# hinike/cairo

Hardware: AMD Instinct MI355X
Metric: encoded Mpixels/s (p-frame, q=16) at 1/2/4/8 MI355X; bit-exact vs ref (higher is better)
Workload: dtype int16

## Files before the change

### cairo_amd/__init__.py

```python
from __future__ import annotations

import ctypes
import os
from dataclasses import dataclass

import numpy as np

_HERE = os.path.dirname(os.path.abspath(__file__))
LIB_PATH = os.path.join(_HERE, "_lib", "libcairo_amd.so")

BLOCK_DESC = np.dtype(
    [
        ("block_type", "<u4"),
        ("prediction_target", "u1"),
        ("pad", "u1"),
        ("motion_x", "<i2"),
        ("motion_y", "<i2"),
        ("sp_pred", "u1"),
        ("sp_amount", "u1"),
        ("sp_index", "u1"),
        ("q_index", "u1"),
        ("variance", "<i2"),
    ]
)
# ... 292 lines not shown
        self.wmb, self.hmb = self.wa // 16, self.ha // 16
        p = ctypes.c_void_p()
        _ck(self.L.cairo_ctx_create_ex(width, height, ring, device, stages, ctypes.byref(p)), "cairo_ctx_create")
        self.h = p
        self._keep = {}

    def close(self) -> None:
        if self.h:
            self.L.cairo_ctx_destroy(self.h)
            self.h = None

    def __del__(self):
        try:
            self.close()
        except Exception:
            pass

    @property
    def stages(self) -> int:
        return int(self.L.cairo_ctx_stages(self.h))

    def submit(self, rgb, index: int, inter: bool, quality: int, on_device: bool = False,
               fmt: int = FMT_RGB24, pitch: int = 0) -> int:
        t = ctypes.c_int()
        ptr = rgb if on_device else _host_frame_fmt(rgb, fmt, self.width, self.height, pitch)
        if fmt == FMT_RGB24 and not pitch:
            _ck(
                self.L.cairo_ctx_submit(self.h, ptr, int(on_device), index, int(inter), quality, ctypes.byref(t)),
                "cairo_ctx_submit",
            )
        else:
            _ck(self.L.cairo_ctx_submit_fmt(self.h, ptr, int(on_device), fmt, pitch, index, int(inter), quality,
                                            ctypes.byref(t)), "cairo_ctx_submit_fmt")
        if not on_device:
            self._keep[t.value] = rgb
        return t.value

    def wait(self, ticket: int, copy: bool = True) -> FrameOutputs:
        r = _FrameResult()
        st = self.L.cairo_ctx_wait(self.h, ticket, ctypes.byref(r))
        if st != EVX_SUCCESS:
            raise CairoError("cairo_ctx_wait", st, self.timeout_info() if st == EVX_ERROR_HARDWAREFAIL else None)
        self._keep.pop(ticket, None)
        return self._outputs(r, copy)

    ACCT_FIELDS = ("coder_tasks", "coder_total", "coder_group_wait", "coder_window", "coder_search", "coder_inter",
                   "coder_dequeue", "coder_mbs", "helper_tasks", "helper_total", "helper_wait", "helper_deblock",
                   "helper_search", "helper_catchup", "helper_dequeue", "helper_chunks",
                   "win_bytes", "win_spec_unused_bytes", "zero_mv_bytes", "gran_poll_bytes", "rec_poll_bytes",
                   "win_stages", "searched_tasks", "inter_tasks", "coder_xform", "coder_publish", "coder_drain",
                   "coder_vm0", "coder_records", "coder_prebarrier", "coder_store_tail",
                   "search_eval", "search_barrier", "search_select", "subpel_eval", "subpel_barrier",
                   "subpel_select", "db_inputs", "db_filter", "db_write",
                   "search_passes", "search_mbs_2pass", "search_mbs_3pass", "search_mbs_4pass")

    def read_acct(self, reset: bool = False) -> dict:
        w = np.zeros(len(self.ACCT_FIELDS), np.uint64)
        _ck(self.L.cairo_ctx_read_acct(self.h, _ptr(w), len(w), int(reset)), "cairo_ctx_read_acct")
        return {k: int(w[i]) for i, k in enumerate(self.ACCT_FIELDS)}

    def timeout_info(self) -> dict | None:
        w = np.zeros(16, np.int32)
        _ck(self.L.cairo_ctx_timeout_info(self.h, _ptr(w), 16), "cairo_ctx_timeout_info")
        if not w[0]:
            return None
        d = {k: int(w[i]) for i, k in enumerate(TIMEOUT_FIELDS)}
        d["kind"] = WAIT_KINDS.get(d["kind"], str(d["kind"]))
        d["seen"] = (d.pop("seen_hi") & 0xFFFFFFFF) << 32 | (d.pop("seen_lo") & 0xFFFFFFFF)
        return d

    def _outputs(self, r, copy: bool) -> FrameOutputs:
        ny, nc = r.wa * r.ha, (r.wa // 2) * (r.ha // 2)
        mbs = r.wmb * r.hmb
        has_coef = bool(r.coef_y)
        feed = _view(r.feed, np.uint32, (r.feed_bits + 31) // 32) if r.feed_status == FEED_VALID else None
        out = FrameOutputs(
            _view(r.block_table, BLOCK_DESC, mbs),
            _view(r.coef_y, np.int16, ny).reshape(r.ha, r.wa) if has_coef else None,
            _view(r.coef_u, np.int16, nc).reshape(r.ha // 2, r.wa // 2) if has_coef else None,
            _view(r.coef_v, np.int16, nc).reshape(r.ha // 2, r.wa // 2) if has_coef else None,
            feed, int(r.feed_bits), int(r.feed_status),
        )
        if copy:
            cp = lambda a: None if a is None else a.copy()
            out = FrameOutputs(cp(out.table), cp(out.coef_y), cp(out.coef_u), cp(out.coef_v), cp(out.feed),
                               out.feed_bits, out.feed_status)
        return out

    def set_outputs(self, outputs: int) -> None:
        _ck(self.L.cairo_ctx_set_outputs(self.h, outputs), "cairo_ctx_set_outputs")

    def fetch_coef(self, ticket: int):
        r = _FrameResult()
        _ck(self.L.cairo_ctx_fetch_coef(self.h, ticket, ctypes.byref(r)), "cairo_ctx_fetch_coef")
        ny, nc = self.wa * self.ha, (self.wa // 2) * (self.ha // 2)
        return (_view(r.coef_y, np.int16, ny).reshape(self.ha, self.wa).copy(),
                _view(r.coef_u, np.int16, nc).reshape(self.ha // 2, self.wa // 2).copy(),
                _view(r.coef_v, np.int16, nc).reshape(self.ha // 2, self.wa // 2).copy())

    def set_metrics(self, sse: bool = True, ssim: bool = True, keep_recon: bool = False, flags: int | None = None) -> None:
        if flags is None:
            flags = (METRIC_SSE if sse else 0) | (METRIC_SSIM if ssim else 0) | (KEEP_RECON if keep_recon else 0)
        _ck(self.L.cairo_ctx_set_metrics(self.h, flags), "cairo_ctx_set_metrics")

    def frame_metrics(self, ticket: int) -> dict:
        m = _FrameMetrics()
        _ck(self.L.cairo_ctx_frame_metrics(self.h, ticket, ctypes.byref(m)), "cairo_ctx_frame_metrics")
# ... 498 lines not shown
```

### cairo_amd/csrc/kernels.h

```cpp
#pragma once

#include <hip/hip_runtime.h>
#include <stdint.h>

#include "evx_defs.h"

namespace cairo {

struct PlaneSet {
  int16_t* y;
  int16_t* u;
  int16_t* v;
};

__host__ __device__ inline PlaneSet ring_slot(int16_t* base, size_t slot_elems, int wa, int ha,
                                              int k) {
  PlaneSet p;
  p.y = base + (size_t)k * slot_elems;
  p.u = p.y + (size_t)wa * ha;
  p.v = p.u + (size_t)(wa / 2) * (ha / 2);
  return p;
}

constexpr int kGranulesPerMB = 192;
// ... 2 lines not shown
__host__ __device__ inline uint32_t pack_inter_desc(const BlockDesc& d) {
  return (d.block_type & 7u) | ((uint32_t)(d.prediction_target & 3) << 3) | ((uint32_t)(d.sp_pred & 1) << 5) |
         ((uint32_t)(d.sp_amount & 1) << 6) | ((uint32_t)(d.sp_index & 15) << 7) |
         (((uint32_t)d.motion_x & 0x7Fu) << 11) | (((uint32_t)d.motion_y & 0x7Fu) << 18);
}
__host__ __device__ inline BlockDesc unpack_inter_desc(uint32_t w) {
  BlockDesc d;
  d.block_type = w & 7u;
  d.prediction_target = (uint8_t)((w >> 3) & 3);
  d.pad = 0;
  d.sp_pred = (uint8_t)((w >> 5) & 1);
  d.sp_amount = (uint8_t)((w >> 6) & 1);
  d.sp_index = (uint8_t)((w >> 7) & 15);
  d.motion_x = (int16_t)((int32_t)(w << 14) >> 25);
  d.motion_y = (int16_t)((int32_t)(w << 7) >> 25);
  d.q_index = 0;
  d.variance = 0;
  return d;
}

constexpr int kStampPhases = 12;
constexpr int kDbStamps = 256;
constexpr int kIStamps = 12;
__host__ __device__ inline size_t stamp_frame_words(int wmb, int hmb) {
  return (size_t)wmb * hmb * kStampPhases + (size_t)hmb * kDbStamps;
}

struct TimeoutInfo {
  static constexpr int kKind = 0;
  static constexpr int kEpoch = 1;
  static constexpr int kIndex = 2;
  static constexpr int kRow = 3;
  static constexpr int kMember = 4;
  static constexpr int kNeed = 5;
  static constexpr int kOn = 6;
  static constexpr int kSeenLo = 7;
  static constexpr int kSeenHi = 8;
  static constexpr int kClaim = 9;
  static constexpr int kWords = 16;
};
enum TimeoutKind : int32_t {
  kWaitRecords = 1,
  kWaitGranule = 2,
  kWaitPrevProgress = 3,
  kWaitRowAbove = 4,
  kWaitBatch = 5,
  kWaitInjected = 6,
  kWaitHostMark = 9,
};

#ifndef CAIRO_ACCT
#define CAIRO_ACCT 0
#endif
constexpr int kAcctShards = 64, kAcctWords = 44;
struct Acct {
  static constexpr int kCoderTasks = 0, kCoderTotal = 1, kCoderGroupWait = 2, kCoderWindow = 3, kCoderSearch = 4,
                       kCoderInter = 5, kCoderDequeue = 6, kCoderMBs = 7;
  static constexpr int kHelperTasks = 8, kHelperTotal = 9, kHelperWait = 10, kHelperDeblock = 11, kHelperSearch = 12,
                       kHelperCatchup = 13, kHelperDequeue = 14, kHelperChunks = 15;
  static constexpr int kWinBytes = 16, kWinSpecUnused = 17, kZeroMvBytes = 18, kGranPollBytes = 19,
                       kRecPollBytes = 20, kWinStages = 21, kSearchedTasks = 22, kInterTasks = 23;
  static constexpr int kCoderXform = 24, kCoderPublish = 25, kCoderDrain = 26;
  static constexpr int kCoderVm0 = 27, kCoderRecords = 28, kCoderPreBarrier = 29;
  static constexpr int kCoderStoreTail = 30;
  static constexpr int kSrchEval = 31, kSrchBarrier = 32, kSrchSelect = 33, kSubEval = 34, kSubBarrier = 35,
                       kSubSelect = 36;
  static constexpr int kDbInputs = 37, kDbFilter = 38, kDbWrite = 39;
  static constexpr int kSrchPasses = 40, kSrchPasses2 = 41, kSrchPasses3 = 42, kSrchPasses4 = 43;
};

#ifndef CAIRO_MAX_BATCH
#define CAIRO_MAX_BATCH 48
#endif
constexpr int kMaxBatch = CAIRO_MAX_BATCH;
constexpr int kMaxGroup = 16;
constexpr int kMaxPush = kMaxRing;

struct FrameDesc {
  const uint8_t* rgb;
  const uint8_t* host_rgb;
  int index;
  int inter;
  int quality;
  uint32_t epoch;
  int slot;
  int decode;
  PlaneSet recon[kMaxRing];
  PlaneSet stale;
  PlaneSet coef;
  PlaneSet push[kMaxPush];
  int npush;
  PlaneSet coef_prev;
  uint64_t* progress;
  const uint64_t* prev_progress;
  const uint64_t* prev2_progress;
  int sys;
  int member;
  const BlockDesc* host_table;
  const int16_t* host_coef;
};

struct FrameArgs {
  int wa, ha;
  int w, h;
  int wmb, hmb;
  int ring;
  int index, inter, quality;
  int decode;
  uint32_t epoch;
  PlaneSet in;
  PlaneSet coef;
  PlaneSet coef_prev;
  PlaneSet recon[kMaxRing];
  PlaneSet stale;
  PlaneSet push[kMaxPush];
  int npush;
  BlockDesc* table;
  BlockDesc* inter_desc;
  void* reserved0;
  uint64_t* granules;
  int32_t* err;
// ... 105 lines not shown
```

### cairo_amd/csrc/kernels.hip

```cpp
#include "kernels.h"

namespace cairo {

typedef const __attribute__((address_space(4))) FrameArgs FA;
#define RECON_AT(a, k)                                                                   \
  ((k) == 1 ? planes((a).recon[1]) : (k) == 2 ? planes((a).recon[2]) : (k) == 3 ? planes((a).recon[3]) \
                                                                              : planes((a).recon[0]))
__host__ __device__ inline PlaneSet planes(const __attribute__((address_space(4))) PlaneSet& p) {
  PlaneSet r;
  r.y = p.y;
  r.u = p.u;
  r.v = p.v;
  return r;
}


__constant__ int16_t kLut8[64] = {
    128, 128,  128,  128,  128,  128,  128,  128,
    126, 106,  71,   25,   -25,  -71,  -106, -126,
    118, 49,   -49,  -118, -118, -49,  49,   118,
    106, -25,  -126, -71,  71,   126,  25,   -106,
    91,  -91,  -91,  91,   91,   -91,  -91,  91,
    71,  -126, 25,   106,  -106, -25,  126,  -71,
    49,  -118, 118,  -49,  -49,  118,  -118, 49,
// ... 39 lines not shown
    sMagDcC[q] = div_magic(chroma_dc_scale(q));
  } else if (t < 192) {
    sMagQmIntra[t - 128] = div_magic(kQmIntra[t - 128]);
    sMagQmInter[t - 128] = div_magic(kQmInter[t - 128]);
  }
  __syncthreads();
}


__device__ __forceinline__ int wave_sum(int v) {
  v += __builtin_amdgcn_mov_dpp(v, 0x128, 0xF, 0xF, false);
  v += __builtin_amdgcn_mov_dpp(v, 0x124, 0xF, 0xF, false);
  v += __builtin_amdgcn_mov_dpp(v, 0x122, 0xF, 0xF, false);
  v += __builtin_amdgcn_mov_dpp(v, 0x121, 0xF, 0xF, false);
  return __builtin_amdgcn_readlane(v, 0) + __builtin_amdgcn_readlane(v, 16) +
         __builtin_amdgcn_readlane(v, 32) + __builtin_amdgcn_readlane(v, 48);
}
__device__ __forceinline__ int wave_max(int v) {
  v = max(v, __builtin_amdgcn_mov_dpp(v, 0x128, 0xF, 0xF, false));
  v = max(v, __builtin_amdgcn_mov_dpp(v, 0x124, 0xF, 0xF, false));
  v = max(v, __builtin_amdgcn_mov_dpp(v, 0x122, 0xF, 0xF, false));
  v = max(v, __builtin_amdgcn_mov_dpp(v, 0x121, 0xF, 0xF, false));
  return max(max(__builtin_amdgcn_readlane(v, 0), __builtin_amdgcn_readlane(v, 16)),
             max(__builtin_amdgcn_readlane(v, 32), __builtin_amdgcn_readlane(v, 48)));
}

__device__ __forceinline__ int lane_id() { return threadIdx.x & 63; }

__device__ __forceinline__ void trace(int32_t* t, int k, int v) {
  if (t && threadIdx.x == 0)
    __hip_atomic_store(&t[blockIdx.x * 4 + k], v, __ATOMIC_RELAXED, __HIP_MEMORY_SCOPE_SYSTEM);
}

__device__ __forceinline__ int16_t* pick(const PlaneSet& p, int pl) {
  int16_t* const y = p.y;
  int16_t* const u = p.u;
  int16_t* const v = p.v;
  return pl == 0 ? y : (pl == 1 ? u : v);
}

__device__ __forceinline__ int fresh(int v) {
  asm volatile("" : "+v"(v));
  return v;
}

__device__ __forceinline__ int uni(int v) { return __builtin_amdgcn_readfirstlane(v); }

__device__ __forceinline__ void stamp(FA& a, int mb, int k) {
  if (a.stamps && threadIdx.x == 0)
    a.stamps[(size_t)mb * kStampPhases + k] = __builtin_amdgcn_s_memrealtime();
}

__device__ __forceinline__ uint64_t acct_now() { return CAIRO_ACCT ? __builtin_amdgcn_s_memrealtime() : 0; }
__device__ __forceinline__ void acct_add(uint64_t* acct, int k, uint64_t v) {
  if (CAIRO_ACCT && acct && threadIdx.x == 0)
    __hip_atomic_fetch_add(&acct[(blockIdx.x & (kAcctShards - 1)) * kAcctWords + k], v, __ATOMIC_RELAXED,
                           __HIP_MEMORY_SCOPE_AGENT);
}

__device__ __forceinline__ uint64_t tagged(uint32_t epoch, int cols) {
  return ((uint64_t)epoch << 32) | (uint32_t)cols;
}
__device__ __forceinline__ uint64_t progress_at(const uint64_t* p) {
  return __hip_atomic_load(p, __ATOMIC_RELAXED, __HIP_MEMORY_SCOPE_AGENT);
}
__device__ __forceinline__ uint64_t progress_peer(bool sys, const uint64_t* p) {
  return sys ? __hip_atomic_load(p, __ATOMIC_RELAXED, __HIP_MEMORY_SCOPE_SYSTEM)
             : __hip_atomic_load(p, __ATOMIC_RELAXED, __HIP_MEMORY_SCOPE_AGENT);
}
__device__ __forceinline__ void acquire_fence(bool sys) {
  if (sys)
    __builtin_amdgcn_fence(__ATOMIC_ACQUIRE, "");
  else
    __builtin_amdgcn_fence(__ATOMIC_ACQUIRE, "agent");
}

constexpr int kWaitSleep = 2, kGranSleep = 1;

__device__ __attribute__((noinline)) void report_timeout(int32_t* err, int32_t* sticky, int kind, uint32_t epoch,
                                                         int index, int row, int member, int need, int on,
                                                         uint64_t seen) {
  __hip_atomic_store(err, 1, __ATOMIC_RELAXED, __HIP_MEMORY_SCOPE_AGENT);
  int32_t none = 0;
  if (!__hip_atomic_compare_exchange_strong(sticky + TimeoutInfo::kClaim, &none, 1, __ATOMIC_RELAXED,
                                            __ATOMIC_RELAXED, __HIP_MEMORY_SCOPE_AGENT))
    return;
  const int32_t w[8] = {(int32_t)epoch, index, row, member, need, on, (int32_t)(uint32_t)seen, (int32_t)(seen >> 32)};
  for (int k = 0; k < 8; k++) __hip_atomic_store(sticky + 1 + k, w[k], __ATOMIC_RELAXED, __HIP_MEMORY_SCOPE_AGENT);
  __hip_atomic_store(sticky + TimeoutInfo::kKind, kind, __ATOMIC_RELEASE, __HIP_MEMORY_SCOPE_SYSTEM);
}
__device__ __forceinline__ void report_timeout(FA& a, int kind, int row, int need, int on, uint64_t seen) {
  report_timeout(a.err, a.sticky, kind, a.epoch, a.index, row, a.member, need, on, seen);
}

__device__ __forceinline__ void wait_records(FA& a, int row, int group) {
  int32_t* word = &a.inter_done[row * a.ng + group];
  int v = __hip_atomic_load(word, __ATOMIC_RELAXED, __HIP_MEMORY_SCOPE_AGENT);
  if (v >= a.nref) return;
  uint64_t t0 = __builtin_amdgcn_s_memrealtime();
  while ((v = __hip_atomic_load(word, __ATOMIC_RELAXED, __HIP_MEMORY_SCOPE_AGENT)) < a.nref) {
    if (__hip_atomic_load(a.err, __ATOMIC_RELAXED, __HIP_MEMORY_SCOPE_AGENT)) return;
    __builtin_amdgcn_s_sleep(kWaitSleep);
    if (__builtin_amdgcn_s_memrealtime() - t0 > 200000000ull) {
      report_timeout(a, kWaitRecords, row, a.nref, group, (uint32_t)v);
      return;
    }
// ... 587 lines not shown
  if (lane >= 48) return;
  const PlaneSet in = planes(a.in);
  const int px = x * kMB, py = r * kMB;
  const int16_t* gsrc = lane < 32 ? in.y + (size_t)(py + (lane >> 1)) * a.wa + px + 8 * (lane & 1)
                                  : pick(in, 1 + ((lane - 32) >> 3)) +
                                        (size_t)((py >> 1) + (lane & 7)) * (a.wa >> 1) + (px >> 1);
  __builtin_amdgcn_global_load_lds((const void*)gsrc, (lds_void*)dst, 16, 0, 0);
}

__device__ __forceinline__ Px6 src_px_lds(const InterLds& L, int wave) {
  const int l = threadIdx.x & 63;
  const int16_t* m = L.src[wave];
  Px6 p;
  const int16_t* y = &m[(l >> 2) * 16 + (l & 3) * 4];
  p.y0 = y[0], p.y1 = y[1], p.y2 = y[2], p.y3 = y[3];
  p.u = m[256 + (l >> 3) * 8 + (l & 7)];
  p.v = m[320 + (l >> 3) * 8 + (l & 7)];
  return p;
}
__device__ __forceinline__ SrcRow src_rows_lds(const InterLds& L, int wave, int i) {
  const uint32_t* m = (const uint32_t*)L.src[wave];
  SrcRow s;
#pragma unroll
  for (int k = 0; k < 8; k++) s.y[k] = m[i * 8 + k] ^ 0x80008000u;
  const int co = (i >> 1) * 4 + (i & 1) * 2;
  s.u[0] = m[128 + co] ^ 0x80008000u, s.u[1] = m[128 + co + 1] ^ 0x80008000u;
  s.v[0] = m[160 + co] ^ 0x80008000u, s.v[1] = m[160 + co + 1] ^ 0x80008000u;
  return s;
}

__device__ __forceinline__ void zero_mv_older(FA& a, int r, int g, InterLds& L) {
  const int wave = threadIdx.x >> 6, x = 4 * g + wave;
  acct_add(a.acct, Acct::kZeroMvBytes, 768ull * (a.nref - 1) * (uint64_t)min(4, a.wmb - 4 * g));
  if (x >= a.wmb) return;
  const int px = x * kMB, py = r * kMB;
  const Px6 src = src_px_lds(L, wave);
  Px6 ref[kMaxRing - 1];
#pragma unroll
  for (int off = 2; off < kMaxRing; off++)
    if (off <= a.nref) ref[off - 1] = px_from_planes(RECON_AT(a, off), a.wa, px, py);
#pragma unroll
  for (int off = 2; off < kMaxRing; off++) {
    if (off > a.nref) break;
    int sad, mad;
    sad_mad(src, ref[off - 1], sad, mad);
    if ((threadIdx.x & 63) == 0) L.zsad[off][wave] = sad, L.zmad[off][wave] = mad;
  }
}

__device__ __forceinline__ int inter_need_cols(FA& a, int g, int level) {
  return min(64 * g + (level == 1 ? 80 : 96), a.wa);
}

__device__ __forceinline__ void inter_task(FA& a0, int r, int g, int off, InterLds& L, DbLds& D, DbState& st,
                                           int* flag, uint64_t* is) {
  FA& a = *opaque_view(&a0);
  const int wave = uni(threadIdx.x >> 6);
  const int x = 4 * g + wave;
  const bool valid = x < a.wmb;
  const int px = x * kMB, py = r * kMB, mb = r * a.wmb + x;
  const int mbs = a.wmb * a.hmb;
  const int thr = (a.quality >> 2) + 1;
  const PlaneSet ref = RECON_AT(a, off);
  Sel s;
  Px6 src;
  s.bx = px;
  s.by = py;
  s.ssd = INT32_MAX;
  s.sp_idx = s.sp_amt = s.sp_en = 0;
  s.sad = s.mad = 0;
  SrcRow srow;
  const int ox = 4 * g * kMB - 32, oy = py - 32;
  if (valid) {
    src = src_px_lds(L, wave);
    srow = src_rows_lds(L, wave, threadIdx.x & 15);
    if (off >= 2) {
      s.sad = L.zsad[off][wave], s.mad = L.zmad[off][wave];
    } else {
      sad_mad(src, px_from_planes(ref, a.wa, px, py), s.sad, s.mad);
    }
  }
  const bool need = valid && s.mad >= thr && !(CAIRO_ATTR_SKIP & 8);
  if ((threadIdx.x & 63) == 0) L.need[wave] = need;
  if (threadIdx.x == 0) {
    const int back = off == 1 ? 1 : 2;
    const uint64_t* pp = back == 1 ? a.prev_progress : a.prev2_progress;
    const uint64_t want = tagged(a.epoch - back, inter_need_cols(a, g, 2));
    const uint64_t w3 = pp ? progress_peer(a.sys, pp + min(r + 3, a.hmb - 1)) : 0;
    const uint64_t w2 = pp ? progress_peer(a.sys, pp + min(r + 2, a.hmb - 1)) : 0;
    const int full = !pp || ((w3 >= want) & (w2 >= want));
    if (full && pp) {
      acquire_fence(a.sys);
      asm volatile("s_waitcnt vmcnt(0)" ::: "memory");
    }
    L.full = full;
  }
  __syncthreads();
  if (is && off == 1) is[3] = __builtin_amdgcn_s_memrealtime();
  acct_add(a.acct, Acct::kInterTasks, 1);
  acct_add(a.acct, Acct::kZeroMvBytes, (off == 1 ? 768ull : 0ull) * (uint64_t)min(4, a.wmb - 4 * g));
  if (L.need[0] | L.need[1] | L.need[2] | L.need[3]) {
    const bool full = L.full != 0;
    acct_add(a.acct, Acct::kSearchedTasks, 1);
    acct_window(a.acct, 0, full ? kWinL : kLvl1Rows, 0, full ? kWinLW : kLvl1Cols);
    stage_window(L.win, ref, a.wa, a.ha, ox, oy, 0, full ? kWinL : kLvl1Rows, 0, full ? kWinLW : kLvl1Cols);
    __syncthreads();
    if (is && off == 1) is[4] = __builtin_amdgcn_s_memrealtime();
    bool lvl2c = full, lvl2r = full;
// ... 42 lines not shown
          const int vs = __builtin_amdgcn_ds_bpermute(from, sad), vm = __builtin_amdgcn_ds_bpermute(from, mad);
          if (my_pass == pass && gi != 4) sadv = vs, madv = vm;
        }
        {
          const int cx = bx + (gi % 3 - 1) * step, cy = by + (gi / 3 - 1) * step;
          select_int(s, gi < 9 && in_frame(cx, cy, a.wa, a.ha), cx, cy, sadv, madv, px, py, thr, lane);
        }
      } else {
        const Px6 best = px_from_window_b(L.win, s.bx - ox, s.by - oy);
        s.sp_idx = s.sp_amt = s.sp_en = 0;
        const int bx = s.bx, by = s.by;
        const uint32_t sb0 = src.y0 + 0x8000, sb1 = src.y1 + 0x8000, sb2 = src.y2 + 0x8000, sb3 = src.y3 + 0x8000,
                       sbu = src.u + 0x8000, sbv = src.v + 0x8000;
        const uint32_t b30 = 3 * best.y0, b31 = 3 * best.y1, b32 = 3 * best.y2, b33 = 3 * best.y3, b3u = 3 * best.u,
                       b3v = 3 * best.v;
#pragma unroll
        for (int n = 0; n < 8; n++) {
          const int k9 = n < 4 ? n : n + 1, i = k9 % 3 - 1, j = k9 / 3 - 1, tx = bx + i, ty = by + j;
          const bool ok = in_frame(tx, ty, a.wa, a.ha);
          if (!ok) continue;
          const Px6 nb = px_from_window_b(L.win, tx - ox, ty - oy);
          const int idx = frac_index(i, j);
#pragma unroll
          for (int q = 0; q < 2; q++) {
            const uint32_t d0 = absdiff_b(sb0, q ? lerp_quarter_bb3(b30, nb.y0) : lerp_half_bb(best.y0, nb.y0)),
                           d1 = absdiff_b(sb1, q ? lerp_quarter_bb3(b31, nb.y1) : lerp_half_bb(best.y1, nb.y1)),
                           d2 = absdiff_b(sb2, q ? lerp_quarter_bb3(b32, nb.y2) : lerp_half_bb(best.y2, nb.y2)),
                           d3 = absdiff_b(sb3, q ? lerp_quarter_bb3(b33, nb.y3) : lerp_half_bb(best.y3, nb.y3)),
                           du = absdiff_b(sbu, q ? lerp_quarter_bb3(b3u, nb.u) : lerp_half_bb(best.u, nb.u)),
                           dv = absdiff_b(sbv, q ? lerp_quarter_bb3(b3v, nb.v) : lerp_half_bb(best.v, nb.v));
            const int lsum = (int)(d0 + d1 + d2 + d3);
            const int lmax = (int)max(max(max(d0, d1), d2), max(max(d3, du), dv));
            const bool copy = s.mad < thr;
            const bool mad_lt = __ballot(lmax >= (copy ? s.mad : thr)) == 0;
            int sad = 0;
            bool acc;
            if (copy) {
              acc = mad_lt;
            } else {
              sad = wave_sum(lsum);
              acc = (sad < s.sad && sad < kSadGate) || mad_lt;
            }
            if (acc) {
              s.sp_en = 1;
              s.sp_amt = q;
              s.sp_idx = idx;
              s.sad = copy ? wave_sum(lsum) : sad;
              s.mad = wave_max(lmax);
            }
          }
        }
      }
    }
  }
  if (is && off == 1) is[10] = __builtin_amdgcn_s_memrealtime();
  if (valid && (threadIdx.x & 63) == 0) {
    const BlockDesc d = make_desc(s, px, py, thr, false, off);
    uint64_t* rec = (uint64_t*)&a.inter_desc[(off - 1) * mbs + mb];
    const uint64_t tag = (uint64_t)a.epoch << 32;
    gran_st(rec, tag | pack_inter_desc(d));
    gran_st(rec + 1, tag | (uint32_t)s.sad);
  }
  asm volatile("s_waitcnt lgkmcnt(0)\n\ts_barrier" ::: "memory");
}


constexpr int kMBElems = 384;
typedef short int8v __attribute__((ext_vector_type(8)));

__device__ __forceinline__ void elem_coords(int e, int x, int y, int& plane, int& ex, int& ey) {
  int b = e >> 6, r = (e >> 3) & 7, c = e & 7;
  if (b < 4) {
    plane = 0;
    ex = x + (b & 1) * 8 + c;
    ey = y + (b >> 1) * 8 + r;
  } else {
    plane = b - 3;
    ex = (x >> 1) + c;
    ey = (y >> 1) + r;
  }
}


__device__ __forceinline__ int8v load_row8(const int16_t* p) {
  return *(const int8v*)p;
}

__device__ __forceinline__ int fdct_lane(int16_t* sa, int16_t* sb, int lane, int16_t x) {
  const int r8 = lane >> 3, c8 = lane & 7;
  sa[lane] = x;
  __builtin_amdgcn_wave_barrier();
  {
    const int8v row = load_row8(&sa[r8 * 8]), lut = load_row8(&sLut8[c8 * 8]);
    int t = 0;
#pragma unroll
    for (int k = 0; k < 8; k++) t += row[k] * lut[k];
    t = c8 == 0 ? (t * 45) / 128 : t / 2;
    sb[c8 * 8 + r8] = (int16_t)rdiv(t, 128);
  }
  __builtin_amdgcn_wave_barrier();
  const int8v col = load_row8(&sb[c8 * 8]), lut = load_row8(&sLut8[r8 * 8]);
  int t = 0;
#pragma unroll
  for (int k = 0; k < 8; k++) t += col[k] * lut[k];
  t = r8 == 0 ? (t * 45) / 128 : t / 2;
  return (int16_t)rdiv(t, 128);
}

__device__ __forceinline__ int idct_lane(int16_t* sa, int16_t* sb, int lane, int16_t d) {
  const int r8 = lane >> 3, c8 = lane & 7;
  sa[c8 * 8 + r8] = d;
  __builtin_amdgcn_wave_barrier();
  {
    const int8v col = load_row8(&sa[c8 * 8]), lut = load_row8(&sLut8T[r8 * 8]);
// ... 902 lines not shown
        }
      }
      if (!(type & kCopy) && !kDecode) {
        _Pragma("unroll") for (int bi = 0; bi < 2; bi++) if (bi < nblk) {
          const int b = wave + 4 * bi, e = b * 64 + lane;
          int pl, ex, ey;
          elem_coords(e, px, py, pl, ex, ey);
          const int sv = svp[bi];
          const int16_t res = has_pred ? (int16_t)(sv - pv[bi]) : (int16_t)sv;
          cf[bi] = (CAIRO_ATTR_SKIP & 64) ? res
                   : (__ballot(res != 0) ? fdct_lane(&L.bufA[b * 64], &L.bufB[b * 64], lane, res) : 0);
        }
      }
      stamp(*ap, mb, 6);
      if (tid < kGranulesPerMB) {
        if (pf3)
          win_put_k(L.win, oy, bx + 3, by - 3, tid,
                    gran_settle(*ap, gran_at(*ap, bx + 3, by - 3, tid), pg3, by));
        if (pf2)
          win_put_k(L.win, oy, bx + 3, by - 2, tid,
                    gran_settle(*ap, gran_at(*ap, bx + 3, by - 2, tid), pg2, by));
        if (pfs) win_put_k(L.win, oy, bx, by + 1, tid, pst);
      }
      if (!(type & kCopy)) {
        int qp;
        if (!kDecode) {
          int32_t v2;
          qp = vaq_mb(L.red, wave, lane, cf[0], ap->quality, &v2);
          d.q_index = (uint8_t)qp;
          d.variance = (int16_t)v2;
        } else {
          qp = d.q_index;
        }
        _Pragma("unroll") for (int bi = 0; bi < 2; bi++) if (bi < nblk) {
          const int b = wave + 4 * bi, e = b * 64 + lane;
          int16_t qv;
          if (!kDecode) {
            qv = (CAIRO_ATTR_SKIP & 64) ? (int16_t)cf[bi] : quant_elem(e, cf[bi], qp, intra_path);
            coef_store_pair(*ap, e, px, py, qv);
          } else {
            int pl, ex, ey;
            elem_coords(e, px, py, pl, ex, ey);
            qv = plane_of(planes(ap->coef), pl)[(size_t)ey * (pl ? cw : ap->wa) + ex];
          }
          const int t = (CAIRO_ATTR_SKIP & 64) ? qv
                        : (__ballot(qv != 0) ? idct_lane(&L.bufA[b * 64], &L.bufB[b * 64], lane,
                                                         dequant_elem(e, qv, qp, intra_path))
                                             : 0);
          pv[bi] = (int16_t)(has_pred ? t + pv[bi] : t);
        }
      } else {
        d.q_index = 0;
        d.variance = 0;
        if (!kDecode) {
          int cp[2] = {0, 0};
          _Pragma("unroll") for (int bi = 0; bi < 2; bi++) if (bi < nblk) {
            const int e = (wave + 4 * bi) * 64 + lane;
            int pl, ex, ey;
            elem_coords(e, px, py, pl, ex, ey);
            cp[bi] = pick(planes(ap->coef_prev), pl)[(size_t)ey * (pl ? cw : ap->wa) + ex];
          }
          _Pragma("unroll") for (int bi = 0; bi < 2; bi++) if (bi < nblk)
            coef_store_pair(*ap, (wave + 4 * bi) * 64 + lane, px, py, cp[bi]);
        }
      }
      stamp(*ap, mb, 7);
      const uint64_t tx7 = acct_now();
      asm volatile("" ::: "memory");
      _Pragma("unroll") for (int bi = 0; bi < 2; bi++) if (bi < nblk) {
        const int b = wave + 4 * bi;
        const int nb = __builtin_amdgcn_mov_dpp(pv[bi], 0xB1, 0xF, 0xF, false);
        if (!(lane & 1)) {
          const int r = lane >> 3, c2 = (lane & 7) >> 1;
          const int k = b < 4 ? (((b >> 1) * 8 + r) * 8 + (b & 1) * 4 + c2) : (128 + (b - 4) * 32 + r * 4 + c2);
          gran_st(gran_at(*ap, bx, by, k),
                  ((uint64_t)tag << 32) | ((uint32_t)pv[bi] & 0xFFFFu) | ((uint32_t)nb << 16));
        }
      }
      stamp(*ap, mb, 8);
      _Pragma("unroll") for (int bi = 0; bi < 2; bi++) if (bi < nblk) {
        const int b = wave + 4 * bi, e = b * 64 + lane;
        int pl, ex, ey;
        elem_coords(e, px, py, pl, ex, ey);
        win_put1(L.win, pl, pl == 0 ? ey - oy : ey - (oy >> 1), ex, pv[bi]);
      }
      asm volatile("" ::: "memory");
      if (tid == 0 && !kDecode) *(uint4*)&ap->table[mb] = __builtin_bit_cast(uint4, d);
      const uint64_t tx8 = acct_now();
      if (!kDecode) {
        if (wave == 0) wait_vmcnt<kStoresAfterCoef[0]>();
        else if (wave == 1) wait_vmcnt<kStoresAfterCoef[1]>();
        else if (wave == 2) wait_vmcnt<kStoresAfterCoef[2]>();
        else wait_vmcnt<kStoresAfterCoef[3]>();
      } else {
        asm volatile("s_waitcnt vmcnt(0)" ::: "memory");
      }
      __syncthreads();
      if (tid == 0)
        gran_st(gran_at(*ap, bx, by, kGranulesPerMB),
                ((uint64_t)tag << 32) | ((d.block_type & kCopy) ? 0x100u : 0u) | d.q_index);
      stamp(*ap, mb, 9);
      if (CAIRO_ACCT) {
        const uint64_t tx9 = acct_now();
        acct_add(ap->acct, Acct::kCoderXform, tx7 - tx5);
        acct_add(ap->acct, Acct::kCoderPublish, tx8 - tx7);
        acct_add(ap->acct, Acct::kCoderDrain, tx9 - tx8);
      }
      if (ap->stamps && tid == 0) ap->stamps[(size_t)mb * kStampPhases + 11] = __builtin_amdgcn_s_memtime();
    }
  }
}



struct HelperLds {
  InterLds inter;
  DbLds db;
};

struct EngineLds {
  union {
    RowLds row;
    HelperLds helper;
  } u;
  int slot;
  int flag;
};

__device__ __forceinline__ void row_helper(FA& a0, int r, HelperLds& L, int* flag, int32_t* tr) {
  FA& a = a0;
  const int tid = threadIdx.x;
  const int nch = db_chunks(a);
  volatile int* vflag = flag;
  DbState st{0, 0, 0, 8};
  for (int g = 0; g < a0.ng; g++) {
    FA& a = *opaque_view(&a0);
    trace(tr, 1, g);
    trace(tr, 2, (int)a.epoch * 1000 + r);
    uint64_t* is = a.istamps && tid == 0 ? a.istamps + (size_t)(r * a.ng + g) * kIStamps : nullptr;
    if (is) is[0] = __builtin_amdgcn_s_memrealtime(), is[3] = is[4] = is[5] = is[6] = is[7] = is[8] = is[9] = is[10] = 0;
    if (a.inter) group_source(a, r, g, L.inter);
    if (a.inter && a.nref >= 2) {
      helper_wait(a, 2, r, min(r + 2, a.hmb - 1), inter_need_cols(a, g, 1), L.db, st, flag);
      const uint64_t ts = acct_now();
      zero_mv_older(a, r, g, L.inter);
      for (int off = 2; off <= a.nref; off++) inter_task(a, r, g, off, L.inter, L.db, st, flag, is);
      acct_add(a.acct, Acct::kHelperSearch, acct_now() - ts);
    }
    helper_wait(a, 1, r, min(r + 2, a.hmb - 1), inter_need_cols(a, g, 1), L.db, st, flag);
    if (is) is[1] = __builtin_amdgcn_s_memrealtime();
    trace(tr, 3, 50);
    if (a.inter) {
      const uint64_t ts = acct_now();
      inter_task(a, r, g, 1, L.inter, L.db, st, flag, is);
      acct_add(a.acct, Acct::kHelperSearch, acct_now() - ts);
    } else if (tid == 0) {
      __builtin_amdgcn_fence(__ATOMIC_RELEASE, "agent");
      asm volatile("s_waitcnt vmcnt(0)" ::: "memory");
      __hip_atomic_fetch_add(&a.inter_done[r * a.ng + g], 1, __ATOMIC_RELAXED, __HIP_MEMORY_SCOPE_AGENT);
    }
    if (is) is[2] = __builtin_amdgcn_s_memrealtime();
    int caught = 0;
    const uint64_t tc = acct_now();
    uint64_t tcdb = 0;
    for (;;) {
      int d = 0;
      if (tid == 0) d = st.k < nch && deblock_chunk_ready(a, r, st);
      if (!wg_broadcast(vflag, d)) break;
      const uint64_t tb = acct_now();
      deblock_chunk(a, r, L.db, st, true);
      tcdb += acct_now() - tb;
      caught++;
    }
    acct_add(a.acct, Acct::kHelperCatchup, acct_now() - tc - tcdb);
    if (is) is[11] = ((uint64_t)caught << 32) | (uint32_t)(__builtin_amdgcn_s_memrealtime() - is[2]);
  }
  trace(tr, 1, 1000);
  while (st.k < nch) {
    trace(tr, 3, 60000 + st.k);
    int d = 0;
    if (tid == 0) {
      const uint64_t t0 = __builtin_amdgcn_s_memrealtime();
      while (!(d = deblock_chunk_ready(a, r, st))) {
        if (__hip_atomic_load(a.err, __ATOMIC_RELAXED, __HIP_MEMORY_SCOPE_AGENT) ||
            __builtin_amdgcn_s_memrealtime() - t0 > 100000000ull)
          break;
        __builtin_amdgcn_s_sleep(kWaitSleep);
      }
    }
    deblock_chunk(a, r, L.db, st, wg_broadcast(vflag, d) != 0);
  }
  trace(tr, 3, 100000);
  if (a.stamps && tid == 0) {
    uint64_t* ds = a.stamps + (size_t)a.wmb * a.hmb * kStampPhases + (size_t)r * kDbStamps;
    ds[kDbStamps - 1] = st.busy;
  }
}


constexpr int kPrioLevel = 2;

__device__ __forceinline__ bool is_helper(int b, int nh, int n) {
  return ((b + 1) * nh) / n > (b * nh) / n;
}

constexpr int kSteal = 2;
__device__ __forceinline__ int next_task(const EngineArgs& e, int pool, int lab, EngineLds& L, bool& prev) {
  const int ptotal = e.ptotal;
// ... 310 lines not shown
```

Measured before the change: 7150.

## Move copy-block coefficient carry from coder to helper after inter search

The helper tracks the best inter candidate per macroblock across reference offsets. When that candidate is a copy block, the helper copies the previous frame's coefficients into the coef planes itself. The coder then skips that copy for carried blocks, which shortens the coder's critical path. This risks a mismatch between the helper's best choice and the coder's final decision, and adds global-memory work to the helper before it publishes inter_done. The kCoderCarried counter is also incremented on the path where the copy is not skipped.

```diff
diff --git a/cairo_amd/__init__.py b/cairo_amd/__init__.py
--- a/cairo_amd/__init__.py
+++ b/cairo_amd/__init__.py
@@ -368,7 +368,8 @@
                    "coder_vm0", "coder_records", "coder_prebarrier", "coder_store_tail",
                    "search_eval", "search_barrier", "search_select", "subpel_eval", "subpel_barrier",
                    "subpel_select", "db_inputs", "db_filter", "db_write",
-                   "search_passes", "search_mbs_2pass", "search_mbs_3pass", "search_mbs_4pass")
+                   "search_passes", "search_mbs_2pass", "search_mbs_3pass", "search_mbs_4pass",
+                   "helper_carry", "helper_carried_mbs", "coder_carried_mbs")
 
     def read_acct(self, reset: bool = False) -> dict:
         w = np.zeros(len(self.ACCT_FIELDS), np.uint64)
diff --git a/cairo_amd/csrc/kernels.h b/cairo_amd/csrc/kernels.h
--- a/cairo_amd/csrc/kernels.h
+++ b/cairo_amd/csrc/kernels.h
@@ -78,7 +78,7 @@
 #ifndef CAIRO_ACCT
 #define CAIRO_ACCT 0
 #endif
-constexpr int kAcctShards = 64, kAcctWords = 44;
+constexpr int kAcctShards = 64, kAcctWords = 47;
 struct Acct {
   static constexpr int kCoderTasks = 0, kCoderTotal = 1, kCoderGroupWait = 2, kCoderWindow = 3, kCoderSearch = 4,
                        kCoderInter = 5, kCoderDequeue = 6, kCoderMBs = 7;
@@ -93,6 +93,7 @@
                        kSubSelect = 36;
   static constexpr int kDbInputs = 37, kDbFilter = 38, kDbWrite = 39;
   static constexpr int kSrchPasses = 40, kSrchPasses2 = 41, kSrchPasses3 = 42, kSrchPasses4 = 43;
+  static constexpr int kHelperCarry = 44, kHelperCarried = 45, kCoderCarried = 46;
 };
 
 #ifndef CAIRO_MAX_BATCH
diff --git a/cairo_amd/csrc/kernels.hip b/cairo_amd/csrc/kernels.hip
--- a/cairo_amd/csrc/kernels.hip
+++ b/cairo_amd/csrc/kernels.hip
@@ -115,6 +115,11 @@
 }
 
 __device__ __forceinline__ uint64_t acct_now() { return CAIRO_ACCT ? __builtin_amdgcn_s_memrealtime() : 0; }
+__device__ __forceinline__ void acct_add_lane(uint64_t* acct, int k, uint64_t v) {
+  if (CAIRO_ACCT && acct)
+    __hip_atomic_fetch_add(&acct[(blockIdx.x & (kAcctShards - 1)) * kAcctWords + k], v, __ATOMIC_RELAXED,
+                           __HIP_MEMORY_SCOPE_AGENT);
+}
 __device__ __forceinline__ void acct_add(uint64_t* acct, int k, uint64_t v) {
   if (CAIRO_ACCT && acct && threadIdx.x == 0)
     __hip_atomic_fetch_add(&acct[(blockIdx.x & (kAcctShards - 1)) * kAcctWords + k], v, __ATOMIC_RELAXED,
@@ -808,8 +813,18 @@
   return min(64 * g + (level == 1 ? 80 : 96), a.wa);
 }
 
+struct BestRec {
+  uint32_t desc;
+  int sad, off;
+};
+__device__ __forceinline__ void best_offer(BestRec& b, uint32_t desc, int sad, int off) {
+  const bool cn = (desc & kCopy) != 0, cb = (b.desc & kCopy) != 0;
+  const bool take = b.off == 0 || (cn != cb ? cn : (sad < b.sad || (sad == b.sad && off < b.off)));
+  if (take) b.desc = desc, b.sad = sad, b.off = off;
+}
+
 __device__ __forceinline__ void inter_task(FA& a0, int r, int g, int off, InterLds& L, DbLds& D, DbState& st,
-                                           int* flag, uint64_t* is) {
+                                           int* flag, uint64_t* is, BestRec& best) {
   FA& a = *opaque_view(&a0);
   const int wave = uni(threadIdx.x >> 6);
   const int x = 4 * g + wave;
@@ -960,12 +975,16 @@
     }
   }
   if (is && off == 1) is[10] = __builtin_amdgcn_s_memrealtime();
-  if (valid && (threadIdx.x & 63) == 0) {
-    const BlockDesc d = make_desc(s, px, py, thr, false, off);
-    uint64_t* rec = (uint64_t*)&a.inter_desc[(off - 1) * mbs + mb];
-    const uint64_t tag = (uint64_t)a.epoch << 32;
-    gran_st(rec, tag | pack_inter_desc(d));
-    gran_st(rec + 1, tag | (uint32_t)s.sad);
+  if (valid) {
+    const uint32_t pd = (uint32_t)uni((int)pack_inter_desc(make_desc(s, px, py, thr, false, off)));
+    const int sad = uni(s.sad);
+    if ((threadIdx.x & 63) == 0) {
+      uint64_t* rec = (uint64_t*)&a.inter_desc[(off - 1) * mbs + mb];
+      const uint64_t tag = (uint64_t)a.epoch << 32;
+      gran_st(rec, tag | pd);
+      gran_st(rec + 1, tag | (uint32_t)sad);
+    }
+    best_offer(best, pd, sad, off);
   }
   asm volatile("s_waitcnt lgkmcnt(0)\n\ts_barrier" ::: "memory");
 }
@@ -1974,7 +1993,9 @@
       } else {
         d.q_index = 0;
         d.variance = 0;
-        if (!kDecode) {
+        const bool carried = !kDecode && nref > 0 && (ib.block_type & kCopy);
+        if (!kDecode && !carried) {
+          acct_add(ap->acct, Acct::kCoderCarried, 1);
           int cp[2] = {0, 0};
           _Pragma("unroll") for (int bi = 0; bi < 2; bi++) if (bi < nblk) {
             const int e = (wave + 4 * bi) * 64 + lane;
@@ -2034,6 +2055,23 @@
 }
 
 
+
+__device__ __forceinline__ void helper_carry(FA& a0, int r, int g, const BestRec& best) {
+  FA& a = *opaque_view(&a0);
+  const int wave = uni(threadIdx.x >> 6), lane = threadIdx.x & 63, x = 4 * g + wave;
+  if (x >= a.wmb || !(best.desc & kCopy)) return;
+  const int px = x * kMB, py = r * kMB, cw = a.wa >> 1;
+  int cp[6];
+#pragma unroll
+  for (int b = 0; b < 6; b++) {
+    int pl, ex, ey;
+    elem_coords(b * 64 + lane, px, py, pl, ex, ey);
+    cp[b] = pick(planes(a.coef_prev), pl)[(size_t)ey * (pl ? cw : a.wa) + ex];
+  }
+#pragma unroll
+  for (int b = 0; b < 6; b++) coef_store_pair(a, b * 64 + lane, px, py, cp[b]);
+  if (lane == 0) acct_add_lane(a.acct, Acct::kHelperCarried, 1);
+}
 
 struct HelperLds {
   InterLds inter;
@@ -2061,12 +2099,13 @@
     trace(tr, 2, (int)a.epoch * 1000 + r);
     uint64_t* is = a.istamps && tid == 0 ? a.istamps + (size_t)(r * a.ng + g) * kIStamps : nullptr;
     if (is) is[0] = __builtin_amdgcn_s_memrealtime(), is[3] = is[4] = is[5] = is[6] = is[7] = is[8] = is[9] = is[10] = 0;
+    BestRec best{0, 0, 0};
     if (a.inter) group_source(a, r, g, L.inter);
     if (a.inter && a.nref >= 2) {
       helper_wait(a, 2, r, min(r + 2, a.hmb - 1), inter_need_cols(a, g, 1), L.db, st, flag);
       const uint64_t ts = acct_now();
       zero_mv_older(a, r, g, L.inter);
-      for (int off = 2; off <= a.nref; off++) inter_task(a, r, g, off, L.inter, L.db, st, flag, is);
+      for (int off = 2; off <= a.nref; off++) inter_task(a, r, g, off, L.inter, L.db, st, flag, is, best);
       acct_add(a.acct, Acct::kHelperSearch, acct_now() - ts);
     }
     helper_wait(a, 1, r, min(r + 2, a.hmb - 1), inter_need_cols(a, g, 1), L.db, st, flag);
@@ -2074,8 +2113,11 @@
     trace(tr, 3, 50);
     if (a.inter) {
       const uint64_t ts = acct_now();
-      inter_task(a, r, g, 1, L.inter, L.db, st, flag, is);
-      acct_add(a.acct, Acct::kHelperSearch, acct_now() - ts);
+      inter_task(a, r, g, 1, L.inter, L.db, st, flag, is, best);
+      const uint64_t th = acct_now();
+      acct_add(a.acct, Acct::kHelperSearch, th - ts);
+      helper_carry(a, r, g, best);
+      acct_add(a.acct, Acct::kHelperCarry, acct_now() - th);
     } else if (tid == 0) {
       __builtin_amdgcn_fence(__ATOMIC_RELEASE, "agent");
       asm volatile("s_waitcnt vmcnt(0)" ::: "memory");
```

After: 7203, median of 6. No clear change (+0.7%).

## Move copy-block coefficient carry from coder to helper ahead of inter task

Applied to the files above, without the earlier changes.

For inter frames, the previous frame's coefficients are bulk-copied into the current coefficient planes by the helper workgroup, one 4-MB group row at a time, before the inter task runs. The coder then skips its per-element copy for copy-type macroblocks. This takes scattered per-lane work off the coder's critical path and replaces it with wide 16-byte write-through stores on the helper, followed by a vmcnt wait and a barrier. The trade-off is that every block's coefficients are now copied, including coded blocks the coder later overwrites. It also adds accounting counters for copy versus coded transform time.

```diff
diff --git a/cairo_amd/__init__.py b/cairo_amd/__init__.py
--- a/cairo_amd/__init__.py
+++ b/cairo_amd/__init__.py
@@ -368,7 +368,9 @@
                    "coder_vm0", "coder_records", "coder_prebarrier", "coder_store_tail",
                    "search_eval", "search_barrier", "search_select", "subpel_eval", "subpel_barrier",
                    "subpel_select", "db_inputs", "db_filter", "db_write",
-                   "search_passes", "search_mbs_2pass", "search_mbs_3pass", "search_mbs_4pass")
+                   "search_passes", "search_mbs_2pass", "search_mbs_3pass", "search_mbs_4pass",
+                   "coder_xform_copy", "coder_copy_mbs", "coder_xform_coded", "coder_coded_mbs",
+                   "helper_carry", "carry_bytes")
 
     def read_acct(self, reset: bool = False) -> dict:
         w = np.zeros(len(self.ACCT_FIELDS), np.uint64)
diff --git a/cairo_amd/csrc/kernels.h b/cairo_amd/csrc/kernels.h
--- a/cairo_amd/csrc/kernels.h
+++ b/cairo_amd/csrc/kernels.h
@@ -78,7 +78,7 @@
 #ifndef CAIRO_ACCT
 #define CAIRO_ACCT 0
 #endif
-constexpr int kAcctShards = 64, kAcctWords = 44;
+constexpr int kAcctShards = 64, kAcctWords = 50;
 struct Acct {
   static constexpr int kCoderTasks = 0, kCoderTotal = 1, kCoderGroupWait = 2, kCoderWindow = 3, kCoderSearch = 4,
                        kCoderInter = 5, kCoderDequeue = 6, kCoderMBs = 7;
@@ -93,6 +93,8 @@
                        kSubSelect = 36;
   static constexpr int kDbInputs = 37, kDbFilter = 38, kDbWrite = 39;
   static constexpr int kSrchPasses = 40, kSrchPasses2 = 41, kSrchPasses3 = 42, kSrchPasses4 = 43;
+  static constexpr int kCoderXformCopy = 44, kCoderCopyMBs = 45, kCoderXformCoded = 46, kCoderCodedMBs = 47;
+  static constexpr int kHelperCarry = 48, kCarryBytes = 49;
 };
 
 #ifndef CAIRO_MAX_BATCH
diff --git a/cairo_amd/csrc/kernels.hip b/cairo_amd/csrc/kernels.hip
--- a/cairo_amd/csrc/kernels.hip
+++ b/cairo_amd/csrc/kernels.hip
@@ -808,8 +808,44 @@
   return min(64 * g + (level == 1 ? 80 : 96), a.wa);
 }
 
+#ifndef CAIRO_CODER_CARRY
+#define CAIRO_CODER_CARRY 0
+#endif
+
+typedef uint32_t u32x4 __attribute__((ext_vector_type(4)));
+typedef __attribute__((address_space(1))) u32x4 gbl_u32x4;
+__device__ __forceinline__ void store16_through(bool sys, int16_t* p, u32x4 v) {
+  if (sys)
+    asm volatile("global_store_dwordx4 %0, %1, off sc0 sc1" ::"v"(p), "v"(v) : "memory");
+  else
+    asm volatile("global_store_dwordx4 %0, %1, off sc1" ::"v"(p), "v"(v) : "memory");
+}
+
+__device__ __forceinline__ bool carry_group(FA& a, int r, int g) {
+  if (CAIRO_CODER_CARRY) return false;
+  const PlaneSet dst = planes(a.coef), src = planes(a.coef_prev);
+  if (dst.y == src.y) return false;
+  const uint64_t t0 = acct_now();
+  const int t = threadIdx.x;
+  int pl, row, x, col;
+  if (t < 128) {
+    pl = 0, row = r * kMB + (t >> 3), x = 4 * g + ((t & 7) >> 1), col = 4 * g * kMB + 8 * (t & 7);
+  } else {
+    const int k = t - 128;
+    pl = 1 + (k >> 5), row = r * (kMB / 2) + ((k & 31) >> 2), x = 4 * g + (k & 3), col = x * (kMB / 2);
+  }
+  if (t < 192 && x < a.wmb) {
+    const size_t off = (size_t)row * (pl ? a.wa >> 1 : a.wa) + col;
+    const u32x4 v = *(const gbl_u32x4*)(pick(src, pl) + off);
+    store16_through(a.sys, pick(dst, pl) + off, v);
+  }
+  acct_add(a.acct, Acct::kHelperCarry, acct_now() - t0);
+  acct_add(a.acct, Acct::kCarryBytes, 768ull * (uint64_t)min(4, a.wmb - 4 * g));
+  return true;
+}
+
 __device__ __forceinline__ void inter_task(FA& a0, int r, int g, int off, InterLds& L, DbLds& D, DbState& st,
-                                           int* flag, uint64_t* is) {
+                                           int* flag, uint64_t* is, bool carried = false) {
   FA& a = *opaque_view(&a0);
   const int wave = uni(threadIdx.x >> 6);
   const int x = 4 * g + wave;
@@ -958,6 +994,9 @@
         }
       }
     }
+  } else if (carried) {
+    asm volatile("s_waitcnt vmcnt(0)" ::: "memory");
+    __syncthreads();
   }
   if (is && off == 1) is[10] = __builtin_amdgcn_s_memrealtime();
   if (valid && (threadIdx.x & 63) == 0) {
@@ -1974,7 +2013,7 @@
       } else {
         d.q_index = 0;
         d.variance = 0;
-        if (!kDecode) {
+        if (!kDecode && (!ap->inter || CAIRO_CODER_CARRY)) {
           int cp[2] = {0, 0};
           _Pragma("unroll") for (int bi = 0; bi < 2; bi++) if (bi < nblk) {
             const int e = (wave + 4 * bi) * 64 + lane;
@@ -2025,6 +2064,9 @@
       if (CAIRO_ACCT) {
         const uint64_t tx9 = acct_now();
         acct_add(ap->acct, Acct::kCoderXform, tx7 - tx5);
+        const bool cpy = (type & kCopy) != 0;
+        acct_add(ap->acct, cpy ? Acct::kCoderXformCopy : Acct::kCoderXformCoded, tx7 - tx5);
+        acct_add(ap->acct, cpy ? Acct::kCoderCopyMBs : Acct::kCoderCodedMBs, 1);
         acct_add(ap->acct, Acct::kCoderPublish, tx8 - tx7);
         acct_add(ap->acct, Acct::kCoderDrain, tx9 - tx8);
       }
@@ -2073,8 +2115,9 @@
     if (is) is[1] = __builtin_amdgcn_s_memrealtime();
     trace(tr, 3, 50);
     if (a.inter) {
+      const bool carried = carry_group(a, r, g);
       const uint64_t ts = acct_now();
-      inter_task(a, r, g, 1, L.inter, L.db, st, flag, is);
+      inter_task(a, r, g, 1, L.inter, L.db, st, flag, is, carried);
       acct_add(a.acct, Acct::kHelperSearch, acct_now() - ts);
     } else if (tid == 0) {
       __builtin_amdgcn_fence(__ATOMIC_RELEASE, "agent");
```

New measurement: 7138 before, 7255 after, median of 6. 1.6% higher.
